# Herong1212/ORB_SLAM3_comments_ghr

Measured on AMD Instinct MI355X. Metric: Mmatches/s (256-bit Hamming), higher is better.
Workload: dtype fp4(e2m1)->f32; 1 GPU; C2: brute-force 256-bit Hamming top-2, 2000 x 2000 descriptors per frame, 1024 independent frames per launch per GPU (headline; the one-frame launch is `sing...; nq=2000, nt=2000, global_batch=1024, parallelism=replicas x1 (independent frames per GPU, no data-path collective)

## Files before the change

### orb_slam3_comments_ghr_amd/csrc/hamming_mfma.hip

```cpp
#include <algorithm>
#include <cstdlib>

#include "osg_internal.h"
#include "top2_key.h"
#include "top2_ring.h"

namespace {

typedef int i32x4 __attribute__((ext_vector_type(4)));
typedef int i32x16 __attribute__((ext_vector_type(16)));

constexpr int MF_PAD = 1 << 30;
constexpr int MF_RS = 272;

__device__ __forceinline__ int med3_i32(int a, int b, int c)
{
    return max(min(a, b), min(max(a, b), c));
}

__device__ __forceinline__ uint32_t spread_query(uint32_t nib)
{
    const uint32_t s = __umul24(nib, 0x204081u) & 0x01010101u;
    return ((0x80808080u - s) & 0x80808080u) | 0x40404040u;
}

__device__ __forceinline__ void key_push(int &k1, int &k2, int key)
{
    k2 = med3_i32(k1, key, k2);
    k1 = min(k1, key);
}

__device__ __forceinline__ void key_push2(int &k1, int &k2, int x, int y)
{
    const int m = med3_i32(k1, x, y);
    k1 = min(min(k1, x), y);
    k2 = min(m, k2);
}

__device__ __forceinline__ void key_push2f(int &k1, int &k2, int x, int y)
{
    const int m = __float_as_int(__builtin_amdgcn_fmed3f(__int_as_float(k1), __int_as_float(x), __int_as_float(y)));
    k1 = min(min(x, y), k1);
    k2 = min(m, k2);
}

__device__ __forceinline__ void key_merge(int &k1, int &k2, int a1, int a2)
{
    const int hi = max(k1, a1);
    k1 = min(k1, a1);
    k2 = min(min(k2, a2), hi);
}

template <int NW, int QT, int CR, int PIPE>
__global__ __launch_bounds__(NW * 64) void k_top2_mfma(const uint32_t *__restrict__ query, int nq,
                                                        const uint32_t *__restrict__ train, int nt,
                                                        int nqb, int32_t *__restrict__ out)
{
    constexpr int NT = NW * 64;
    constexpr int BPT = CR * 32 / NT;
    constexpr int WPT = BPT / 4;
    constexpr int TPR = 32 / BPT;
    constexpr int NTILE = CR / 32;
    static_assert(CR * 32 % NT == 0 && BPT % 4 == 0 && TPR >= 1, "chunk / workgroup shape");
    __shared__ __attribute__((aligned(16))) unsigned char s_buf[2 * CR * MF_RS];
    __shared__ uint2 s_lut[256];

    const int t = threadIdx.x, lane = t & 63;
    const int w = __builtin_amdgcn_readfirstlane(t >> 6);
    const int G = gridDim.x, L = blockIdx.x;
    const int logical = (G % 8 == 0) ? (L % 8) * (G / 8) + L / 8 : L;
    const int b = logical / nqb, qb = logical % nqb;
    const uint32_t *qf = query + (size_t)b * nq * 8;
    const uint32_t *tf = train + (size_t)b * nt * 8;
    int32_t *of = out + (size_t)b * nq * 3;

    for (int e = t; e < 256; e += NT) {
        uint32_t lo = 0, hi = 0;
#pragma unroll
        for (int y = 0; y < 4; y++) {
            lo |= ((e >> y) & 1u) << (8 * y + 7);
            hi |= ((e >> (y + 4)) & 1u) << (8 * y + 7);
        }
        s_lut[e] = make_uint2(lo, hi);
    }

    const int r = lane & 31, h = lane >> 5;
    const int qw0 = qb * (NW * QT * 32) + w * (QT * 32);
    const bool active = qw0 < nq;

    i32x4 bq[QT][8];
    int ka1[QT], ka2[QT], kb1[QT], kb2[QT], pq[QT];
#pragma unroll
    for (int j = 0; j < QT; j++) {
        const int q = min(qw0 + 32 * j + r, nq - 1);
        const uint4 lo = *(const uint4 *)(qf + (size_t)q * 8), hi = *(const uint4 *)(qf + (size_t)q * 8 + 4);
        const uint32_t wd[8] = {lo.x, lo.y, lo.z, lo.w, hi.x, hi.y, hi.z, hi.w};
        int pc = 0;
#pragma unroll
        for (int s = 0; s < 8; s++) {
            pc += __popc(wd[s]);
            const uint32_t hw = h ? (wd[s] >> 16) : (wd[s] & 0xFFFFu);
#pragma unroll
            for (int d = 0; d < 4; d++) bq[j][s][d] = (int)spread_query((hw >> (4 * d)) & 0xFu);
        }
        pq[j] = pc;
        ka1[j] = ka2[j] = kb1[j] = kb2[j] = (256 - pc) << MF_SHIFT;
    }
    i32x16 crow;
#pragma unroll
    for (int i = 0; i < 16; i++) crow[i] = (i & 3) + 8 * (i >> 2) + 4 * h;
    const int lbase = r * MF_RS + h * 16;

    const int erow = t / TPR, epart = t % TPR;
    auto load_chunk = [&](int c0, uint32_t (&pw)[WPT]) {
        const int row = c0 + erow;
        if (row < nt) {
            const uint32_t *src = tf + (size_t)row * 8 + epart * WPT;
#pragma unroll
            for (int i = 0; i < WPT; i += 2) {
                const uint2 v = *(const uint2 *)(src + i);
                pw[i] = v.x;
                pw[i + 1] = v.y;
            }
        } else {
#pragma unroll
            for (int i = 0; i < WPT; i++) pw[i] = 0u;
        }
    };
    auto store_chunk = [&](int buf, const uint32_t (&pw)[WPT]) {
        unsigned char *dst = s_buf + ((size_t)buf * CR + erow) * MF_RS;
#pragma unroll
        for (int i = 0; i < WPT; i++) {
#pragma unroll
            for (int hh = 0; hh < 2; hh++) {
                const int g = 2 * (epart * WPT + i) + hh;
                const uint2 v0 = s_lut[(pw[i] >> (16 * hh)) & 0xFFu];
                const uint2 v1 = s_lut[(pw[i] >> (16 * hh + 8)) & 0xFFu];
                *(i32x4 *)(dst + 16 * g) = i32x4{(int)v0.x, (int)v0.y, (int)v1.x, (int)v1.y};
            }
        }
    };

    auto frag = [&](const unsigned char *tb, int s) -> i32x4 { return *(const i32x4 *)(tb + lbase + 32 * s); };
    auto mfma = [&](const i32x4 &a, const i32x4 &bb, const i32x16 &c) {
        return __builtin_amdgcn_mfma_i32_32x32x32_i8(a, bb, c, 0, 0, 0);
    };
    auto epi = [&](const i32x16 (&acc)[QT]) {
#pragma unroll
        for (int j = 0; j < QT; j++) {
#pragma unroll
            for (int i = 0; i < 8; i += 2) {
                key_push2(ka1[j], ka2[j], acc[j][i], acc[j][i + 1]);
                key_push2(kb1[j], kb2[j], acc[j][i + 8], acc[j][i + 9]);
            }
            ka1[j] -= 32;
            ka2[j] -= 32;
            kb1[j] -= 32;
            kb2[j] -= 32;
        }
    };
    auto tile = [&](const unsigned char *tb, const i32x16 &cin) {
        i32x4 a[8];
#pragma unroll
        for (int s = 0; s < 8; s++) a[s] = frag(tb, s);
        i32x16 acc[QT];
#pragma unroll
        for (int j = 0; j < QT; j++) acc[j] = mfma(a[0], bq[j][0], cin);
#pragma unroll
        for (int s = 1; s < 8; s++)
#pragma unroll
            for (int j = 0; j < QT; j++) acc[j] = mfma(a[s], bq[j][s], acc[j]);
        epi(acc);
    };

    const int nch = (nt + CR - 1) / CR;
    {
        uint32_t pw[WPT];
        load_chunk(0, pw);
        __syncthreads();
        store_chunk(0, pw);
    }
    __syncthreads();
    for (int c = 0; c < nch; c++) {
        const int c0 = c * CR;
        uint32_t pw[WPT];
        const bool more = c + 1 < nch;
        if (more) load_chunk(c0 + CR, pw);
        if (active) {
            const unsigned char *sb = s_buf + (size_t)(c & 1) * CR * MF_RS;
            const int nfull = min(NTILE, (nt - c0) / 32);
            if (PIPE && nfull == NTILE) {
                i32x4 a[8];
                i32x16 accp[QT], acc[QT];
#pragma unroll
                for (int s = 0; s < 8; s++) a[s] = frag(sb, s);
#pragma unroll
                for (int s = 0; s < 8; s++) {
#pragma unroll
                    for (int j = 0; j < QT; j++) accp[j] = mfma(a[s], bq[j][s], s ? accp[j] : crow);
                    a[s] = frag(sb + 32 * MF_RS, s);
                    __builtin_amdgcn_sched_barrier(0);
                }
#pragma unroll
                for (int tt = 1; tt < NTILE; tt++) {
#pragma unroll
                    for (int s = 0; s < 8; s++) {
#pragma unroll
                        for (int j = 0; j < QT; j++) acc[j] = mfma(a[s], bq[j][s], s ? acc[j] : crow);
                        if (tt + 1 < NTILE) a[s] = frag(sb + (tt + 1) * 32 * MF_RS, s);
#pragma unroll
                        for (int j = 0; j < QT; j++) {
                            if (s & 1)
                                key_push2(kb1[j], kb2[j], accp[j][8 + (s & 6)], accp[j][9 + (s & 6)]);
                            else
                                key_push2(ka1[j], ka2[j], accp[j][s & 6], accp[j][1 + (s & 6)]);
                            if (s == 7) {
                                ka1[j] -= 32;
                                ka2[j] -= 32;
                                kb1[j] -= 32;
                                kb2[j] -= 32;
                            }
                        }
                        __builtin_amdgcn_sched_barrier(0);
                    }
#pragma unroll
                    for (int j = 0; j < QT; j++) accp[j] = acc[j];
                }
                epi(accp);
            } else {
#pragma unroll
                for (int tt = 0; tt < NTILE; tt++) {
                    if (tt >= nfull) break;
                    tile(sb + tt * 32 * MF_RS, crow);
                }
            }
            const int lim = nt - (c0 + nfull * 32);
            if (nfull < NTILE && lim > 0) {
                i32x16 cin;
#pragma unroll
                for (int i = 0; i < 16; i++) cin[i] = crow[i] + (crow[i] >= lim ? MF_PAD : 0);
                tile(sb + nfull * 32 * MF_RS, cin);
            }
        }
        if (more) store_chunk((c + 1) & 1, pw);
        __syncthreads();
    }
    if (!active) return;
    const int base = 32 * ((nt + 31) / 32);
#pragma unroll
    for (int j = 0; j < QT; j++) {
        int k1 = ka1[j], k2 = ka2[j];
        key_merge(k1, k2, kb1[j], kb2[j]);
        const int a1 = __shfl_xor(k1, 32), a2 = __shfl_xor(k2, 32);
        key_merge(k1, k2, a1, a2);
        const int q = qw0 + 32 * j + r;
        if (h == 0 && q < nq) {
            const int t1 = k1 + base, t2 = k2 + base;
            const int d1 = (t1 >> MF_SHIFT) + pq[j], d2 = (t2 >> MF_SHIFT) + pq[j];
            of[3 * q + 0] = d1 < 256 ? (t1 & (MF_MAX_ROWS - 1)) : -1;
            of[3 * q + 1] = min(d1, 256);
            of[3 * q + 2] = min(d2, 256);
        }
    }
}

constexpr int MX_RS = 144;
constexpr int MX_SCALE_TRAIN = 127 + 12;
constexpr int MX_SCALE_ONE = 127;
constexpr float MX_BIAS = 10485760.0f;
constexpr float MX_PAD = 1073741824.0f;

typedef int i32x8 __attribute__((ext_vector_type(8)));
typedef float f32x16 __attribute__((ext_vector_type(16)));

__device__ __forceinline__ uint32_t spread_nib(uint32_t x)
{
    x &= 0xFFu;
    x = (x | (x << 12)) & 0x000F000Fu;
    x = (x | (x << 6)) & 0x03030303u;
    return (x | (x << 3)) & 0x11111111u;
}

__device__ __forceinline__ uint32_t spread_nib9(uint32_t x)
{
    uint32_t lo3 = x * 0x40201u;
    asm("" : "+v"(lo3));
    return (lo3 | (x << 27)) & 0x88888888u;
}

template <int NW, int QT, int CR, int PIPE>
__global__ __launch_bounds__(NW * 64) void k_top2_fp4(const uint32_t *__restrict__ query, int nq,
                                                       const uint32_t *__restrict__ train, int nt,
                                                       int nqb, int32_t *__restrict__ out)
{
    constexpr int NT = NW * 64;
    constexpr int BPT = CR * 32 / NT;
    constexpr int WPT = BPT / 4;
    constexpr int TPR = 32 / BPT;
    constexpr int NTILE = CR / 32;
    static_assert(CR * 32 % NT == 0 && BPT % 4 == 0 && TPR >= 1, "chunk / workgroup shape");
    __shared__ __attribute__((aligned(16))) unsigned char s_buf[2 * CR * MX_RS];
    __shared__ uint32_t s_lut[256];

    const int t = threadIdx.x, lane = t & 63;
    const int w = __builtin_amdgcn_readfirstlane(t >> 6);
    const int G = gridDim.x, L = blockIdx.x;
    const int logical = (G % 8 == 0) ? (L % 8) * (G / 8) + L / 8 : L;
    const int b = logical / nqb, qb = logical % nqb;
    const uint32_t *qf = query + (size_t)b * nq * 8;
    const uint32_t *tf = train + (size_t)b * nt * 8;
    int32_t *of = out + (size_t)b * nq * 3;

    for (int e = t; e < 256; e += NT) s_lut[e] = spread_nib((uint32_t)e) * 0xCu;

    const int r = lane & 31, h = lane >> 5;
    const int qw0 = qb * (NW * QT * 32) + w * (QT * 32);
    const bool active = qw0 < nq;

    i32x8 bq[QT][4];
    int ka1[QT], ka2[QT], kb1[QT], kb2[QT];
    constexpr bool ONE = PIPE == 3 || PIPE == 4 || PIPE == 5;
    constexpr bool PART = PIPE == 5;
    int(&kc1)[QT] = ONE ? ka1 : kb1;
    int(&kc2)[QT] = ONE ? ka2 : kb2;
    int pq[QT];
#pragma unroll
    for (int j = 0; j < QT; j++) {
        const int q = min(qw0 + 32 * j + r, nq - 1);
        const uint4 lo = *(const uint4 *)(qf + (size_t)q * 8), hi = *(const uint4 *)(qf + (size_t)q * 8 + 4);
        const uint32_t wd[8] = {lo.x, lo.y, lo.z, lo.w, hi.x, hi.y, hi.z, hi.w};
        int pc = 0;
#pragma unroll
        for (int k = 0; k < 8; k++) pc += __popc(wd[k]);
#pragma unroll
        for (int s = 0; s < 4; s++) {
            const uint32_t word = wd[2 * s + h];
#pragma unroll
            for (int d = 0; d < 4; d++)
                bq[j][s][d] = (int)(0x22222222u | ((~spread_nib(word >> (8 * d)) & 0x11111111u) << 3));
#pragma unroll
            for (int d = 4; d < 8; d++) bq[j][s][d] = 0;
        }
        pq[j] = pc;
        ka1[j] = ka2[j] = kb1[j] = kb2[j] = ((256 - pc) << MF_SHIFT) + MX_KEY0;
    }
    f32x16 crow;
#pragma unroll
    for (int i = 0; i < 16; i++) crow[i] = MX_BIAS + (float)((i & 3) + 8 * (i >> 2) + 4 * h);
    const int lbase = r * MX_RS + h * 16;

    const int erow = t / TPR, epart = t % TPR;
    auto load_chunk = [&](int c0, uint32_t (&pw)[WPT]) {
        const int row = c0 + erow;
        if (row < nt) {
            const uint32_t *src = tf + (size_t)row * 8 + epart * WPT;
#pragma unroll
            for (int i = 0; i < WPT; i += 2) {
                const uint2 v = *(const uint2 *)(src + i);
                pw[i] = v.x;
                pw[i + 1] = v.y;
            }
        } else {
#pragma unroll
            for (int i = 0; i < WPT; i++) pw[i] = 0u;
        }
    };
    auto store_chunk = [&](int buf, const uint32_t (&pw)[WPT]) {
        unsigned char *dst = s_buf + ((size_t)buf * CR + erow) * MX_RS;
#pragma unroll
        for (int i = 0; i < WPT; i++) {
            const uint32_t x = pw[i];
            *(i32x4 *)(dst + 16 * (epart * WPT + i)) =
                i32x4{(int)s_lut[x & 0xFFu], (int)s_lut[(x >> 8) & 0xFFu], (int)s_lut[(x >> 16) & 0xFFu],
                      (int)s_lut[x >> 24]};
        }
    };

    auto frag = [&](const unsigned char *tb, int s) -> i32x8 {
        const i32x4 v = *(const i32x4 *)(tb + lbase + 32 * s);
        return i32x8{v[0], v[1], v[2], v[3], 0, 0, 0, 0};
    };
    auto mfma = [&](const i32x8 &a, const i32x8 &bb, const f32x16 &c) {
        return __builtin_amdgcn_mfma_scale_f32_32x32x64_f8f6f4(a, bb, c, 4, 4, 0, MX_SCALE_TRAIN, 0, MX_SCALE_ONE);
    };
    auto epi = [&](const f32x16 (&acc)[QT]) {
#pragma unroll
        for (int j = 0; j < QT; j++) {
#pragma unroll
            for (int i = 0; i < 8; i += 2) {
                key_push2f(ka1[j], ka2[j], __float_as_int(acc[j][i]), __float_as_int(acc[j][i + 1]));
                key_push2f(kc1[j], kc2[j], __float_as_int(acc[j][i + 8]), __float_as_int(acc[j][i + 9]));
            }
            ka1[j] -= 32;
            ka2[j] -= 32;
            if (!ONE) {
                kb1[j] -= 32;
                kb2[j] -= 32;
            }
        }
    };
    auto tile = [&](const unsigned char *tb, const f32x16 &cin) {
        i32x8 a[4];
#pragma unroll
        for (int s = 0; s < 4; s++) a[s] = frag(tb, s);
        f32x16 acc[QT];
#pragma unroll
        for (int j = 0; j < QT; j++) acc[j] = mfma(a[0], bq[j][0], cin);
#pragma unroll
        for (int s = 1; s < 4; s++)
#pragma unroll
            for (int j = 0; j < QT; j++) acc[j] = mfma(a[s], bq[j][s], acc[j]);
        epi(acc);
    };

    const int nch = (nt + CR - 1) / CR;
    {
        uint32_t pw[WPT];
        load_chunk(0, pw);
        __syncthreads();
        store_chunk(0, pw);
    }
    __syncthreads();
    for (int c = 0; c < nch; c++) {
        const int c0 = c * CR;
        uint32_t pw[WPT];
        const bool more = c + 1 < nch;
        if (more) load_chunk(c0 + CR, pw);
        if (active) {
            const unsigned char *sb = s_buf + (size_t)(c & 1) * CR * MX_RS;
            const int nfull = min(NTILE, (nt - c0) / 32);
            if (PIPE && (nfull == NTILE || (PART && nfull >= 1))) {
                i32x8 a[4];
                f32x16 accp[QT], acc[QT];
#pragma unroll
                for (int s = 0; s < 4; s++) a[s] = frag(sb, s);
#pragma unroll
                for (int s = 0; s < 4; s++) {
#pragma unroll
                    for (int j = 0; j < QT; j++) accp[j] = mfma(a[s], bq[j][s], s ? accp[j] : crow);
                    a[s] = frag(sb + 32 * MX_RS, s);
                    __builtin_amdgcn_sched_barrier(0);
                }
#pragma unroll
                for (int tt = 1; tt < NTILE; tt++) {
                    if (PART && tt >= nfull) break;
#pragma unroll
                    for (int s = 0; s < 4; s++) {
#pragma unroll
                        for (int j = 0; j < QT; j++) acc[j] = mfma(a[s], bq[j][s], s ? acc[j] : crow);
                        if (tt + 1 < NTILE) a[s] = frag(sb + (tt + 1) * 32 * MX_RS, s);
                        if (PIPE == 4) {
                            if (s == 1) {
                                bool need = false;
#pragma unroll
                                for (int j = 0; j < QT; j++) {
                                    int m = __float_as_int(accp[j][0]);
#pragma unroll
                                    for (int e = 1; e < 16; e += 2)
                                        m = min(min(m, __float_as_int(accp[j][e])),
                                                __float_as_int(accp[j][e + 1 < 16 ? e + 1 : e]));
                                    need |= m < ka2[j];
                                }
                                if (__builtin_amdgcn_ballot_w64(need) != 0) {
#pragma unroll
                                    for (int j = 0; j < QT; j++)
#pragma unroll
                                        for (int e = 0; e < 16; e += 2)
                                            key_push2f(ka1[j], ka2[j], __float_as_int(accp[j][e]),
                                                      __float_as_int(accp[j][e + 1]));
                                }
#pragma unroll
                                for (int j = 0; j < QT; j++) {
                                    ka1[j] -= 32;
                                    ka2[j] -= 32;
                                }
                            }
                            __builtin_amdgcn_sched_barrier(0);
                            continue;
                        }
#pragma unroll
                        for (int j = 0; j < QT; j++) {
                            if (PIPE == 2) {
#pragma unroll
                                for (int p = 0; p < 8; p++) {
                                    if (p / 3 + 1 != s) continue;
                                    const int e = (p & 3) * 2 + (p >> 2) * 8;
                                    if (p < 4) key_push2f(ka1[j], ka2[j], __float_as_int(accp[j][e]), __float_as_int(accp[j][e + 1]));
                                    else key_push2f(kb1[j], kb2[j], __float_as_int(accp[j][e]), __float_as_int(accp[j][e + 1]));
                                }
                            } else {
                                key_push2f(ka1[j], ka2[j], __float_as_int(accp[j][2 * s]),
                                          __float_as_int(accp[j][2 * s + 1]));
                                key_push2f(kc1[j], kc2[j], __float_as_int(accp[j][8 + 2 * s]),
                                          __float_as_int(accp[j][9 + 2 * s]));
                            }
                            if (s == 3) {
                                ka1[j] -= 32;
                                ka2[j] -= 32;
                                if (!ONE) {
                                    kb1[j] -= 32;
                                    kb2[j] -= 32;
                                }
                            }
                        }
                        __builtin_amdgcn_sched_barrier(0);
                    }
#pragma unroll
                    for (int j = 0; j < QT; j++) accp[j] = acc[j];
                }
                epi(accp);
            } else {
#pragma unroll
                for (int tt = 0; tt < NTILE; tt++) {
                    if (tt >= nfull) break;
                    tile(sb + tt * 32 * MX_RS, crow);
                }
            }
            const int lim = nt - (c0 + nfull * 32);
            if (nfull < NTILE && lim > 0) {
                f32x16 cin;
#pragma unroll
                for (int i = 0; i < 16; i++)
                    cin[i] = crow[i] + ((i & 3) + 8 * (i >> 2) + 4 * h >= lim ? MX_PAD : 0.f);
                tile(sb + nfull * 32 * MX_RS, cin);
            }
        }
        if (more) store_chunk((c + 1) & 1, pw);
        __syncthreads();
    }
    if (!active) return;
    const int base = 32 * ((nt + 31) / 32);
#pragma unroll
    for (int j = 0; j < QT; j++) {
        int k1 = ka1[j], k2 = ka2[j];
        if (!ONE) key_merge(k1, k2, kb1[j], kb2[j]);
        const int a1 = __shfl_xor(k1, 32), a2 = __shfl_xor(k2, 32);
        key_merge(k1, k2, a1, a2);
        const int q = qw0 + 32 * j + r;
        if (h == 0 && q < nq) {
            const int t1 = k1 - MX_KEY0 + base, t2 = k2 - MX_KEY0 + base;
            const int d1 = (t1 >> MF_SHIFT) + pq[j], d2 = (t2 >> MF_SHIFT) + pq[j];
            of[3 * q + 0] = d1 < 256 ? (t1 & (MF_MAX_ROWS - 1)) : -1;
            of[3 * q + 1] = min(d1, 256);
            of[3 * q + 2] = min(d2, 256);
        }
    }
}

template <int NW, int QT, int CR>
__global__ __launch_bounds__(NW * 64) void k_top2_fp4p(const uint32_t *__restrict__ query, int nq,
                                                        const uint32_t *__restrict__ train, int nt,
                                                        int nqb, int n_items, int32_t *__restrict__ out)
{
    constexpr int NT = NW * 64;
    constexpr int BPT = CR * 32 / NT;
    constexpr int WPT = BPT / 4;
    constexpr int TPR = 32 / BPT;
    constexpr int NTILE = CR / 32;
    static_assert(CR * 32 % NT == 0 && BPT % 4 == 0 && TPR >= 1, "chunk / workgroup shape");
    __shared__ __attribute__((aligned(16))) unsigned char s_buf[2 * CR * MX_RS];
    __shared__ uint32_t s_lut[256];

    const int t = threadIdx.x, lane = t & 63;
    const int w = __builtin_amdgcn_readfirstlane(t >> 6);
    const int G = gridDim.x;
    auto logical_of = [&](int item) { return (n_items % 8 == 0) ? (item % 8) * (n_items / 8) + item / 8 : item; };
    int item = blockIdx.x;
    if (item >= n_items) return;
    for (int e = t; e < 256; e += NT) s_lut[e] = spread_nib((uint32_t)e) * 0xCu;
    const int r = lane & 31, h = lane >> 5;
    const int lbase = r * MX_RS + h * 16;
    const int erow = t / TPR, epart = t % TPR;
    auto load_chunk = [&](const uint32_t *tfp, int c0, uint32_t (&pw)[WPT]) {
        const int row = c0 + erow;
        if (row < nt) {
            const uint32_t *src = tfp + (size_t)row * 8 + epart * WPT;
#pragma unroll
            for (int i = 0; i < WPT; i += 2) {
                const uint2 v = *(const uint2 *)(src + i);
                pw[i] = v.x;
                pw[i + 1] = v.y;
            }
        } else {
#pragma unroll
            for (int i = 0; i < WPT; i++) pw[i] = 0u;
        }
    };
    auto store_chunk = [&](int buf, const uint32_t (&pw)[WPT]) {
        unsigned char *dst = s_buf + ((size_t)buf * CR + erow) * MX_RS;
#pragma unroll
        for (int i = 0; i < WPT; i++) {
            const uint32_t x = pw[i];
            *(i32x4 *)(dst + 16 * (epart * WPT + i)) =
                i32x4{(int)s_lut[x & 0xFFu], (int)s_lut[(x >> 8) & 0xFFu], (int)s_lut[(x >> 16) & 0xFFu],
                      (int)s_lut[x >> 24]};
        }
    };
    auto frag = [&](const unsigned char *tb, int s) -> i32x8 {
        const i32x4 v = *(const i32x4 *)(tb + lbase + 32 * s);
        return i32x8{v[0], v[1], v[2], v[3], 0, 0, 0, 0};
    };
    auto mfma = [&](const i32x8 &a, const i32x8 &bb, const f32x16 &c) {
        return __builtin_amdgcn_mfma_scale_f32_32x32x64_f8f6f4(a, bb, c, 4, 4, 0, MX_SCALE_TRAIN, 0, MX_SCALE_ONE);
    };
    const int nch = (nt + CR - 1) / CR;
    {
        uint32_t pw[WPT];
        load_chunk(train + (size_t)(logical_of(item) / nqb) * nt * 8, 0, pw);
        __syncthreads();
        store_chunk(0, pw);
    }
    __syncthreads();
    int bufbase = 0;
    for (; item < n_items; item += G) {
        const int logical = logical_of(item);
        const int b = logical / nqb, qb = logical % nqb;
        const uint32_t *qf = query + (size_t)b * nq * 8;
        const uint32_t *tf = train + (size_t)b * nt * 8;
        int32_t *of = out + (size_t)b * nq * 3;
        const int next = item + G;
        const uint32_t *tfn = next < n_items ? train + (size_t)(logical_of(next) / nqb) * nt * 8 : nullptr;
        const int qw0 = qb * (NW * QT * 32) + w * (QT * 32);
        const bool active = qw0 < nq;
        i32x8 bq[QT][4];
        int ka1[QT], ka2[QT], pq[QT];
#pragma unroll
        for (int j = 0; j < QT; j++) {
            const int q = min(qw0 + 32 * j + r, nq - 1);
            const uint4 lo = *(const uint4 *)(qf + (size_t)q * 8), hi = *(const uint4 *)(qf + (size_t)q * 8 + 4);
            const uint32_t wd[8] = {lo.x, lo.y, lo.z, lo.w, hi.x, hi.y, hi.z, hi.w};
            int pc = 0;
#pragma unroll
            for (int k = 0; k < 8; k++) pc += __popc(wd[k]);
#pragma unroll
            for (int s = 0; s < 4; s++) {
                const uint32_t word = wd[2 * s + h];
#pragma unroll
                for (int d = 0; d < 4; d++)
                    bq[j][s][d] = (int)(0x22222222u | ((~spread_nib(word >> (8 * d)) & 0x11111111u) << 3));
#pragma unroll
                for (int d = 4; d < 8; d++) bq[j][s][d] = 0;
            }
            pq[j] = pc;
            ka1[j] = ka2[j] = ((256 - pc) << MF_SHIFT) + MX_KEY0;
        }
        f32x16 crow;
#pragma unroll
        for (int i = 0; i < 16; i++) crow[i] = MX_BIAS + (float)((i & 3) + 8 * (i >> 2) + 4 * h);
        auto epi = [&](const f32x16 (&acc)[QT]) {
#pragma unroll
            for (int j = 0; j < QT; j++) {
#pragma unroll
                for (int i = 0; i < 8; i += 2) {
                    key_push2f(ka1[j], ka2[j], __float_as_int(acc[j][i]), __float_as_int(acc[j][i + 1]));
                    key_push2f(ka1[j], ka2[j], __float_as_int(acc[j][i + 8]), __float_as_int(acc[j][i + 9]));
                }
                ka1[j] -= 32;
                ka2[j] -= 32;
            }
        };
        auto tile = [&](const unsigned char *tb, const f32x16 &cin) {
            i32x8 a[4];
#pragma unroll
            for (int s = 0; s < 4; s++) a[s] = frag(tb, s);
            f32x16 acc[QT];
#pragma unroll
            for (int j = 0; j < QT; j++) acc[j] = mfma(a[0], bq[j][0], cin);
#pragma unroll
            for (int s = 1; s < 4; s++)
#pragma unroll
                for (int j = 0; j < QT; j++) acc[j] = mfma(a[s], bq[j][s], acc[j]);
            epi(acc);
        };
        for (int c = 0; c < nch; c++) {
            const int c0 = c * CR;
            uint32_t pw[WPT];
            const bool more_in = c + 1 < nch, more = more_in || tfn != nullptr;
            if (more_in) load_chunk(tf, c0 + CR, pw);
            else if (tfn) load_chunk(tfn, 0, pw);
            if (active) {
                const unsigned char *sb = s_buf + (size_t)((c + bufbase) & 1) * CR * MX_RS;
                const int nfull = min(NTILE, (nt - c0) / 32);
                if (nfull == NTILE) {
                    i32x8 a[4];
                    f32x16 accp[QT], acc[QT];
#pragma unroll
                    for (int s = 0; s < 4; s++) a[s] = frag(sb, s);
#pragma unroll
                    for (int s = 0; s < 4; s++) {
#pragma unroll
                        for (int j = 0; j < QT; j++) accp[j] = mfma(a[s], bq[j][s], s ? accp[j] : crow);
                        a[s] = frag(sb + 32 * MX_RS, s);
                        __builtin_amdgcn_sched_barrier(0);
                    }
#pragma unroll
                    for (int tt = 1; tt < NTILE; tt++) {
#pragma unroll
                        for (int s = 0; s < 4; s++) {
#pragma unroll
                            for (int j = 0; j < QT; j++) acc[j] = mfma(a[s], bq[j][s], s ? acc[j] : crow);
                            if (tt + 1 < NTILE) a[s] = frag(sb + (tt + 1) * 32 * MX_RS, s);
#pragma unroll
                            for (int j = 0; j < QT; j++) {
                                key_push2f(ka1[j], ka2[j], __float_as_int(accp[j][2 * s]),
                                           __float_as_int(accp[j][2 * s + 1]));
                                key_push2f(ka1[j], ka2[j], __float_as_int(accp[j][8 + 2 * s]),
                                           __float_as_int(accp[j][9 + 2 * s]));
                                if (s == 3) {
                                    ka1[j] -= 32;
                                    ka2[j] -= 32;
                                }
                            }
                            __builtin_amdgcn_sched_barrier(0);
                        }
#pragma unroll
                        for (int j = 0; j < QT; j++) accp[j] = acc[j];
                    }
                    epi(accp);
                } else {
#pragma unroll
                    for (int tt = 0; tt < NTILE; tt++) {
                        if (tt >= nfull) break;
                        tile(sb + tt * 32 * MX_RS, crow);
                    }
                }
                const int lim = nt - (c0 + nfull * 32);
                if (nfull < NTILE && lim > 0) {
                    f32x16 cin;
#pragma unroll
                    for (int i = 0; i < 16; i++)
                        cin[i] = crow[i] + ((i & 3) + 8 * (i >> 2) + 4 * h >= lim ? MX_PAD : 0.f);
                    tile(sb + nfull * 32 * MX_RS, cin);
                }
            }
            if (more) store_chunk((c + 1 + bufbase) & 1, pw);
            __syncthreads();
        }
        bufbase = (bufbase + nch) & 1;
        if (active) {
            const int base = 32 * ((nt + 31) / 32);
#pragma unroll
            for (int j = 0; j < QT; j++) {
                int k1 = ka1[j], k2 = ka2[j];
                const int a1 = __shfl_xor(k1, 32), a2 = __shfl_xor(k2, 32);
                key_merge(k1, k2, a1, a2);
                const int q = qw0 + 32 * j + r;
                if (h == 0 && q < nq) {
                    const int t1 = k1 - MX_KEY0 + base, t2 = k2 - MX_KEY0 + base;
                    const int d1 = (t1 >> MF_SHIFT) + pq[j], d2 = (t2 >> MF_SHIFT) + pq[j];
                    of[3 * q + 0] = d1 < 256 ? (t1 & (MF_MAX_ROWS - 1)) : -1;
                    of[3 * q + 1] = min(d1, 256);
                    of[3 * q + 2] = min(d2, 256);
                }
            }
        }
    }
}

template <int NW, int CR>
__global__ __launch_bounds__(NW * 64) void k_top2_fp4q2(const uint32_t *__restrict__ query, int nq,
                                                         const uint32_t *__restrict__ train, int nt,
                                                         int nqb, int32_t *__restrict__ out)
{
    constexpr int NT = NW * 64;
    constexpr int BPT = CR * 32 / NT;
    constexpr int WPT = BPT / 4;
    constexpr int TPR = 32 / BPT;
    constexpr int NTILE = CR / 32;
    static_assert(CR * 32 % NT == 0 && BPT % 8 == 0 && TPR >= 1, "chunk / workgroup shape");
    constexpr int SLOTB = CR * MX_RS;
    __shared__ __attribute__((aligned(16))) unsigned char s_mem[1024 + TOP2_RING_SLOTS * SLOTB];
    uint32_t *const s_lut = (uint32_t *)s_mem;
    unsigned char *const s_buf = s_mem + 1024;

    const int t = threadIdx.x, lane = t & 63;
    const int w = __builtin_amdgcn_readfirstlane(t >> 6);
    const int G = gridDim.x, L = blockIdx.x;
    const int logical = (G % 8 == 0) ? (L % 8) * (G / 8) + L / 8 : L;
    const int b = logical / nqb, qb = logical % nqb;
    const uint32_t *qf = query + (size_t)b * nq * 8;
    const uint32_t *tf = train + (size_t)b * nt * 8;
    int32_t *of = out + (size_t)b * nq * 3;

    for (int e = t; e < 256; e += NT) {
        const uint32_t x = spread_nib9((uint32_t)e);
        s_lut[e] = x | (x >> 1);
    }

    const int r = lane & 31, h = lane >> 5;
    const int qw0 = qb * (NW * 64) + w * 64;
    const bool act0 = qw0 < nq, act1 = qw0 + 32 < nq;

    auto load_chunk = [&](int t, int c0, uint32_t (&pw)[WPT]) {
        const char *src = (const char *)tf + (c0 + t / TPR < nt ? (unsigned)((c0 * 8 + t * WPT) * 4) : 0u);
#pragma unroll
        for (int i = 0; i < WPT; i += 2) {
            const uint2 v = *(const uint2 *)(src + 4 * i);
            pw[i] = v.x;
            pw[i + 1] = v.y;
        }
    };
    uint32_t pw[WPT], p1[WPT];
    load_chunk(t, 0, pw);
    load_chunk(t, CR, p1);

    i32x8 bq[2][4];
    int k1[2], k2[2];
#pragma unroll
    for (int j = 0; j < 2; j++) {
        const int q = min(qw0 + 32 * j + r, nq - 1);
        const uint4 lo = *(const uint4 *)(qf + (size_t)q * 8), hi = *(const uint4 *)(qf + (size_t)q * 8 + 4);
        const int pc = __popc(lo.x) + __popc(lo.y) + __popc(lo.z) + __popc(lo.w) + __popc(hi.x) + __popc(hi.y) +
                       __popc(hi.z) + __popc(hi.w);
        const uint32_t wsel[4] = {h ? lo.y : lo.x, h ? lo.w : lo.z, h ? hi.y : hi.x, h ? hi.w : hi.z};
#pragma unroll
        for (int s = 0; s < 4; s++) {
            const uint32_t word = wsel[s];
#pragma unroll
            for (int d = 0; d < 4; d++)
                bq[j][s][d] = (int)(spread_nib9((word >> (8 * d)) & 0xFFu) ^ 0xAAAAAAAAu);
#pragma unroll
            for (int d = 4; d < 8; d++) bq[j][s][d] = 0;
        }
        k1[j] = k2[j] = ((256 - pc) << MF_SHIFT) + MX_KEY0;
    }
    f32x16 crow;
#pragma unroll
    for (int i = 0; i < 16; i++) crow[i] = MX_BIAS + (float)((i & 3) + 8 * (i >> 2) + 4 * h);
    int lbase = r * MX_RS + h * 16;

    auto store_chunk = [&](int t, int buf, int c0, const uint32_t (&pw)[WPT]) {
        const bool in = c0 + t / TPR < nt;
        unsigned char *dst = s_buf + buf * SLOTB + ((t & (NT - 1)) / TPR) * MX_RS + (t % TPR) * (16 * WPT);
#pragma unroll
        for (int i = 0; i < WPT; i++) {
            const uint32_t x = in ? pw[i] : 0u;
            *(i32x4 *)(dst + 16 * i) =
                i32x4{(int)s_lut[x & 0xFFu], (int)s_lut[(x >> 8) & 0xFFu], (int)s_lut[(x >> 16) & 0xFFu],
                      (int)s_lut[x >> 24]};
        }
    };
    auto frag = [&](const unsigned char *tb, int s) -> i32x8 {
        const i32x4 v = *(const i32x4 *)(tb + lbase + 32 * s);
        return i32x8{v[0], v[1], v[2], v[3], 0, 0, 0, 0};
    };
    auto mfma = [&](const i32x8 &a, const i32x8 &bb, const f32x16 &c) {
        return __builtin_amdgcn_mfma_scale_f32_32x32x64_f8f6f4(a, bb, c, 4, 4, 0, MX_SCALE_TRAIN, 0, MX_SCALE_ONE);
    };
    auto push = [&](int j, const f32x16 &acc, int s) {
        key_push2f(k1[j], k2[j], __float_as_int(acc[2 * s]), __float_as_int(acc[2 * s + 1]));
        key_push2f(k1[j], k2[j], __float_as_int(acc[8 + 2 * s]), __float_as_int(acc[9 + 2 * s]));
        if (s == 3) k1[j] -= TOP2_TILE_ROWS;
    };
    auto pushk = [&](int j, const f32x16 &acc, int s) {
        const int lo = s == 0 ? 0 : 3 * (s - 1), hi = s == 0 ? 0 : (s == 3 ? 8 : 3 * s);
#pragma unroll
        for (int p = lo; p < hi; p++) {
            const int e = (p & 1) * 8 + 2 * (p >> 1);
            key_push2f(k1[j], k2[j], __float_as_int(acc[e]), __float_as_int(acc[e + 1]));
        }
        if (s == 3) k1[j] -= TOP2_TILE_ROWS;
    };
    auto tile = [&](const unsigned char *tb, const f32x16 &cin) {
        i32x8 a[4];
#pragma unroll
        for (int s = 0; s < 4; s++) a[s] = frag(tb, s);
        f32x16 acc0 = mfma(a[0], bq[0][0], cin);
#pragma unroll
        for (int s = 1; s < 4; s++) acc0 = mfma(a[s], bq[0][s], acc0);
        if (act1) {
            f32x16 acc1 = mfma(a[0], bq[1][0], cin);
#pragma unroll
            for (int s = 1; s < 4; s++) acc1 = mfma(a[s], bq[1][s], acc1);
#pragma unroll
            for (int s = 0; s < 4; s++) push(0, acc0, s);
#pragma unroll
            for (int s = 0; s < 4; s++) push(1, acc1, s);
        } else {
#pragma unroll
            for (int s = 0; s < 4; s++) push(0, acc0, s);
        }
    };

    const int nch = top2_ring_chunks(nt, CR), nfc = top2_ring_full_chunks(nt, CR);
    __syncthreads();
    store_chunk(t, top2_ring_slot(0), 0, pw);
    store_chunk(t, top2_ring_slot(1), CR, p1);
    load_chunk(t, TOP2_RING_AHEAD * CR, pw);
    __syncthreads();
    auto lane_again = [&]() {
        int ln;
        asm volatile("v_mbcnt_lo_u32_b32 %0, -1, 0\n\tv_mbcnt_hi_u32_b32 %0, -1, %0" : "=v"(ln));
        return ln & 63;
    };
    auto seam = [&](int c, int freed) {
        __syncthreads();
        const int ln = lane_again(), tv = w * 64 + ln;
        store_chunk(tv, freed, (c + TOP2_RING_AHEAD) * CR, pw);
        load_chunk(tv, (c + TOP2_RING_AHEAD + 1) * CR, pw);
        return ln;
    };
    int slot = top2_ring_slot(0), freed = top2_ring_slot(TOP2_RING_SLOTS - 1);
    if (act1) {
        if (nfc > 0) {
            i32x8 a[4];
            f32x16 acc0, acc1;
#pragma unroll
            for (int s = 0; s < 4; s++) a[s] = frag(s_buf + slot * SLOTB, s);
#pragma unroll
            for (int i = 0; i < 16; i++) acc1[i] = MX_PAD;
            k1[1] += TOP2_TILE_ROWS;
            for (int c = 0; c < nfc; c++) {
#pragma unroll
                for (int s = 0; s < 4; s++) {
                    acc0 = mfma(a[s], bq[0][s], s ? acc0 : crow);
                    __builtin_amdgcn_sched_barrier(0);
                    pushk(1, acc1, s);
                    __builtin_amdgcn_sched_barrier(0);
                }
                const int ln = seam(c, freed);
                const int next = top2_ring_next(slot);
                lbase = (ln & 31) * MX_RS + (ln >> 5) * 16;
                const unsigned char *sb = s_buf + slot * SLOTB, *sn = sb + (next - slot) * SLOTB;
#pragma unroll
                for (int tt = 0; tt < NTILE; tt++) {
                    const unsigned char *nb = tt + 1 < NTILE ? sb + (tt + 1) * 32 * MX_RS : sn;
#pragma unroll
                    for (int s = 0; s < 4; s++) {
                        acc1 = mfma(a[s], bq[1][s], s ? acc1 : crow);
                        a[s] = frag(nb, s);
                        __builtin_amdgcn_sched_barrier(0);
                        pushk(0, acc0, s);
                        __builtin_amdgcn_sched_barrier(0);
                    }
                    if (tt + 1 == NTILE) break;
#pragma unroll
                    for (int s = 0; s < 4; s++) {
                        acc0 = mfma(a[s], bq[0][s], s ? acc0 : crow);
                        __builtin_amdgcn_sched_barrier(0);
                        pushk(1, acc1, s);
                        __builtin_amdgcn_sched_barrier(0);
                    }
                }
                freed = slot;
                slot = next;
            }
#pragma unroll
            for (int s = 0; s < 4; s++) push(1, acc1, s);
        }
    } else {
        for (int c = 0; c < nfc; c++) {
            seam(c, freed);
            if (act0) {
                const int nfull = min(NTILE, (nt - c * CR) / 32);
#pragma unroll 1
                for (int tt = 0; tt < nfull; tt++) tile(s_buf + slot * SLOTB + tt * 32 * MX_RS, crow);
            }
            freed = slot;
            slot = top2_ring_next(slot);
        }
    }
    if (nfc < nch) {
        seam(nfc, freed);
        if (act0) {
            const int ln = (int)__builtin_amdgcn_mbcnt_hi(~0u, __builtin_amdgcn_mbcnt_lo(~0u, 0u)), h = ln >> 5;
            lbase = (ln & 31) * MX_RS + h * 16;
            const unsigned char *sb = s_buf + slot * SLOTB;
            const int c0 = nfc * CR, nfull = (nt - c0) / 32;
#pragma unroll 1
            for (int tt = 0; tt < nfull; tt++) tile(sb + tt * 32 * MX_RS, crow);
            const int lim = nt - (c0 + nfull * 32);
            if (lim > 0) {
                f32x16 cin;
#pragma unroll
                for (int i = 0; i < 16; i++)
                    cin[i] = crow[i] + (4 * h >= lim - ((i & 3) + 8 * (i >> 2)) ? MX_PAD : 0.f);
                tile(sb + nfull * 32 * MX_RS, cin);
            }
        }
    }
    if (!act0) return;
    const int base = 32 * ((nt + 31) / 32);
    const int lane_end = (int)__builtin_amdgcn_mbcnt_hi(~0u, __builtin_amdgcn_mbcnt_lo(~0u, 0u));
#pragma unroll
    for (int j = 0; j < 2; j++) {
        int m1 = k1[j], m2 = k2[j];
        const int a1 = __shfl_xor(m1, 32), a2 = __shfl_xor(m2, 32);
        m2 = min(min(m2, a2), max(m1, a1) + TOP2_K2_LAST_REBASE);
        m1 = min(m1, a1);
        const int q = qw0 + 32 * j + lane_end;
        if (lane_end < 32 && q < nq) {
            const uint4 lo = *(const uint4 *)(qf + (size_t)q * 8), hi = *(const uint4 *)(qf + (size_t)q * 8 + 4);
            const int pc = __popc(lo.x) + __popc(lo.y) + __popc(lo.z) + __popc(lo.w) + __popc(hi.x) + __popc(hi.y) +
                           __popc(hi.z) + __popc(hi.w);
            const int d1 = top2_k1_dist(m1, base) + pc, d2 = top2_k2_dist(m2) + pc;
            of[3 * q + 0] = d1 < 256 ? top2_k1_row(m1, base) : -1;
            of[3 * q + 1] = min(d1, 256);
            of[3 * q + 2] = min(d2, 256);
        }
    }
}

template <int NW, int CR>
int launch_fp4q2(osg_ctx *ctx, const void *d_query, int nq, const void *d_train, int nt, int nb, void *d_out)
{
    const int nqb = (nq + NW * 64 - 1) / (NW * 64);
    const long long g = (long long)nqb * nb;
    OSG_REQUIRE(ctx, g <= 0x7FFFFFFF, "grid too large");
    hipLaunchKernelGGL((k_top2_fp4q2<NW, CR>), dim3((unsigned)g), dim3(NW * 64), 0, ctx->stream,
                       (const uint32_t *)d_query, nq, (const uint32_t *)d_train, nt, nqb, (int32_t *)d_out);
    OSG_HIP_CHECK(ctx, hipGetLastError());
    return OSG_OK;
}

template <int NW, int QT, int CR>
int launch_fp4p(osg_ctx *ctx, const void *d_query, int nq, const void *d_train, int nt, int nb, void *d_out)
{
    const int nqb = (nq + NW * QT * 32 - 1) / (NW * QT * 32);
    const long long items = (long long)nqb * nb;
    OSG_REQUIRE(ctx, items <= 0x7FFFFFFF, "grid too large");
    static int ncu = 0;
    if (ncu == 0) {
        int dev = 0, n = 0;
        if (hipGetDevice(&dev) == hipSuccess && hipDeviceGetAttribute(&n, hipDeviceAttributeMultiprocessorCount, dev) == hipSuccess && n > 0)
            ncu = n;
        else
            ncu = 256;
    }
    const int g = (int)std::min<long long>(items, ncu);
    hipLaunchKernelGGL((k_top2_fp4p<NW, QT, CR>), dim3((unsigned)std::max(g, 1)), dim3(NW * 64), 0, ctx->stream,
                       (const uint32_t *)d_query, nq, (const uint32_t *)d_train, nt, nqb, (int)items, (int32_t *)d_out);
    OSG_HIP_CHECK(ctx, hipGetLastError());
    return OSG_OK;
}

template <int NW, int QT, int CR, int PIPE>
int launch_fp4(osg_ctx *ctx, const void *d_query, int nq, const void *d_train, int nt, int nb, void *d_out)
{
    const int nqb = (nq + NW * QT * 32 - 1) / (NW * QT * 32);
    const long long g = (long long)nqb * nb;
    OSG_REQUIRE(ctx, g <= 0x7FFFFFFF, "grid too large");
    hipLaunchKernelGGL((k_top2_fp4<NW, QT, CR, PIPE>), dim3((unsigned)g), dim3(NW * 64), 0, ctx->stream,
                       (const uint32_t *)d_query, nq, (const uint32_t *)d_train, nt, nqb, (int32_t *)d_out);
    OSG_HIP_CHECK(ctx, hipGetLastError());
    return OSG_OK;
}

template <int NW, int QT, int CR, int PIPE>
int launch(osg_ctx *ctx, const void *d_query, int nq, const void *d_train, int nt, int nb, void *d_out)
{
    const int nqb = (nq + NW * QT * 32 - 1) / (NW * QT * 32);
    const long long g = (long long)nqb * nb;
    OSG_REQUIRE(ctx, g <= 0x7FFFFFFF, "grid too large");
    hipLaunchKernelGGL((k_top2_mfma<NW, QT, CR, PIPE>), dim3((unsigned)g), dim3(NW * 64), 0, ctx->stream,
                       (const uint32_t *)d_query, nq, (const uint32_t *)d_train, nt, nqb, (int32_t *)d_out);
    OSG_HIP_CHECK(ctx, hipGetLastError());
    return OSG_OK;
}

}

int osg_top2_mfma_max_rows() { return MF_MAX_ROWS; }

namespace {
int mfma_shape()
{
    static const int shape = getenv("OSG_TOP2_MFMA_SHAPE") ? atoi(getenv("OSG_TOP2_MFMA_SHAPE")) : 0;
    return shape;
}
bool mfma_fp4()
{
    static const bool fp4 = !(getenv("OSG_TOP2_FP4") && atoi(getenv("OSG_TOP2_FP4")) == 0);
    return fp4;
}
void mfma_shape_of(bool fp4, int shape, int *d)
{
    static const int i8[5][4] = {{16, 1, 256, 1}, {8, 2, 256, 1}, {16, 1, 256, 0}, {8, 2, 256, 0}, {8, 1, 256, 1}};
    static const int f4[14][4] = {{16, 1, 256, 3}, {8, 2, 256, 1}, {16, 1, 256, 0}, {16, 1, 256, 3}, {8, 1, 256, 1},
                                  {16, 2, 256, 1}, {16, 1, 256, 2}, {16, 1, 256, 1}, {16, 1, 256, 4}, {8, 1, 256, 3},
                                  {16, 1, 512, 3}, {16, 1, 256, 5}, {16, 1, 512, 5}, {16, 1, 256, 6}};
    const int *s = fp4 ? f4[(shape >= 1 && shape <= 13 && shape != 3) ? shape : 0]
                       : i8[(shape >= 1 && shape <= 4) ? shape : 0];
    for (int i = 0; i < 4; i++) d[i] = s[i];
}
bool mfma_q2(bool fp4, int shape) { return fp4 && !(shape >= 1 && shape <= 13); }
}

int osg_hamming_top2_batch_plan(osg_ctx *ctx, int32_t nq, int32_t nt, int32_t nb, char *name, int32_t len)
{
    if (!ctx || !name || len <= 0) return OSG_E_INVALID;
    const bool mf = getenv("OSG_TOP2_BATCH_MFMA") == nullptr || atoi(getenv("OSG_TOP2_BATCH_MFMA")) != 0;
    if (nq <= 0 || nb <= 0 || nt <= 0 || !mf || nt > MF_MAX_ROWS) {
        snprintf(name, (size_t)len, "%s", nq <= 0 || nb <= 0 ? "none" : "k_top2_batch");
        return OSG_OK;
    }
    if (mfma_q2(mfma_fp4(), mfma_shape())) {
        snprintf(name, (size_t)len, "k_top2_fp4q2<16,256> grid=%lld x %d", (long long)((nq + 1023) / 1024) * nb, 1024);
        return OSG_OK;
    }
    int d[4];
    mfma_shape_of(mfma_fp4(), mfma_shape(), d);
    const int per_wg = d[0] * d[1] * 32;
    snprintf(name, (size_t)len, "%s<%d,%d,%d,%d> grid=%lld x %d", mfma_fp4() ? "k_top2_fp4" : "k_top2_mfma", d[0], d[1],
             d[2], d[3], (long long)((nq + per_wg - 1) / per_wg) * nb, d[0] * 64);
    return OSG_OK;
}

int osg_launch_top2_batch_mfma(osg_ctx *ctx, const void *d_query, int32_t nq, const void *d_train, int32_t nt,
                               int32_t nb, void *d_out)
{
    OSG_REQUIRE(ctx, nt >= 1 && nt <= MF_MAX_ROWS, "nt=%d outside the MFMA path's 1..%d rows", nt, MF_MAX_ROWS);
    const int shape = mfma_shape();
    if (mfma_fp4()) {
        if (mfma_q2(true, shape)) return launch_fp4q2<16, 256>(ctx, d_query, nq, d_train, nt, nb, d_out);
        switch (shape) {
        case 1: return launch_fp4<8, 2, 256, 1>(ctx, d_query, nq, d_train, nt, nb, d_out);
        case 2: return launch_fp4<16, 1, 256, 0>(ctx, d_query, nq, d_train, nt, nb, d_out);
        case 4: return launch_fp4<8, 1, 256, 1>(ctx, d_query, nq, d_train, nt, nb, d_out);
        case 5: return launch_fp4<16, 2, 256, 1>(ctx, d_query, nq, d_train, nt, nb, d_out);
        case 6: return launch_fp4<16, 1, 256, 2>(ctx, d_query, nq, d_train, nt, nb, d_out);
        case 7: return launch_fp4<16, 1, 256, 1>(ctx, d_query, nq, d_train, nt, nb, d_out);
        case 8: return launch_fp4<16, 1, 256, 4>(ctx, d_query, nq, d_train, nt, nb, d_out);
        case 9: return launch_fp4<8, 1, 256, 3>(ctx, d_query, nq, d_train, nt, nb, d_out);
        case 10: return launch_fp4<16, 1, 512, 3>(ctx, d_query, nq, d_train, nt, nb, d_out);
        case 11: return launch_fp4<16, 1, 256, 5>(ctx, d_query, nq, d_train, nt, nb, d_out);
        case 12: return launch_fp4<16, 1, 512, 5>(ctx, d_query, nq, d_train, nt, nb, d_out);
        case 13: return launch_fp4p<16, 1, 256>(ctx, d_query, nq, d_train, nt, nb, d_out);
        default: return launch_fp4<16, 1, 256, 3>(ctx, d_query, nq, d_train, nt, nb, d_out);
        }
    }
    switch (shape) {
    case 1: return launch<8, 2, 256, 1>(ctx, d_query, nq, d_train, nt, nb, d_out);
    case 2: return launch<16, 1, 256, 0>(ctx, d_query, nq, d_train, nt, nb, d_out);
    case 3: return launch<8, 2, 256, 0>(ctx, d_query, nq, d_train, nt, nb, d_out);
    case 4: return launch<8, 1, 256, 1>(ctx, d_query, nq, d_train, nt, nb, d_out);
    default: return launch<16, 1, 256, 1>(ctx, d_query, nq, d_train, nt, nb, d_out);
    }
}
```

Before: 10.24 million Mmatches/s.

## Use buffer loads for train staging and peel non-prefetch tail chunks

Train-descriptor loads now go through AMD buffer resources whose size bound makes out-of-range reads return zero, so the per-thread bounds check and the zero-select in the store path go away. Staging offsets are precomputed once, the LDS lookup uses a scalar shift, and fragment addressing becomes an integer offset on a single running base instead of re-derived pointers and lane IDs. The main loop is specialised at compile time so the last chunks skip the useless store and prefetch. The MFMA scale operands are packed differently. This trims address and VALU work in the steady-state loop, but it relies on buffer out-of-bounds semantics and on the modified scale encoding staying equivalent.

```diff
diff --git a/orb_slam3_comments_ghr_amd/csrc/hamming_mfma.hip b/orb_slam3_comments_ghr_amd/csrc/hamming_mfma.hip
--- a/orb_slam3_comments_ghr_amd/csrc/hamming_mfma.hip
+++ b/orb_slam3_comments_ghr_amd/csrc/hamming_mfma.hip
@@ -1,5 +1,6 @@
 #include <algorithm>
 #include <cstdlib>
+#include <type_traits>
 
 #include "osg_internal.h"
 #include "top2_key.h"
@@ -791,18 +792,21 @@
     const int qw0 = qb * (NW * 64) + w * 64;
     const bool act0 = qw0 < nq, act1 = qw0 + 32 < nq;
 
-    auto load_chunk = [&](int t, int c0, uint32_t (&pw)[WPT]) {
-        const char *src = (const char *)tf + (c0 + t / TPR < nt ? (unsigned)((c0 * 8 + t * WPT) * 4) : 0u);
+    const unsigned src8 = (unsigned)t * (WPT * 4);
+    const int stg = (t / TPR) * MX_RS + (t % TPR) * (16 * WPT);
+    auto load_chunk = [&](unsigned src8, int c0, uint32_t (&pw)[WPT]) {
+        const __amdgpu_buffer_rsrc_t rs = __builtin_amdgcn_make_buffer_rsrc(
+            (void *)((const char *)tf + (size_t)c0 * 32), 0, max(nt - c0, 0) * 32, 0x00020000);
 #pragma unroll
         for (int i = 0; i < WPT; i += 2) {
-            const uint2 v = *(const uint2 *)(src + 4 * i);
+            const uint2 v = __builtin_bit_cast(uint2, __builtin_amdgcn_raw_buffer_load_b64(rs, (int)src8 + 4 * i, 0, 0));
             pw[i] = v.x;
             pw[i + 1] = v.y;
         }
     };
     uint32_t pw[WPT], p1[WPT];
-    load_chunk(t, 0, pw);
-    load_chunk(t, CR, p1);
+    load_chunk(src8, 0, pw);
+    load_chunk(src8, CR, p1);
 
     i32x8 bq[2][4];
     int k1[2], k2[2];
@@ -829,23 +833,24 @@
     for (int i = 0; i < 16; i++) crow[i] = MX_BIAS + (float)((i & 3) + 8 * (i >> 2) + 4 * h);
     int lbase = r * MX_RS + h * 16;
 
-    auto store_chunk = [&](int t, int buf, int c0, const uint32_t (&pw)[WPT]) {
-        const bool in = c0 + t / TPR < nt;
-        unsigned char *dst = s_buf + buf * SLOTB + ((t & (NT - 1)) / TPR) * MX_RS + (t % TPR) * (16 * WPT);
+    int two;
+    asm("s_mov_b32 %0, 2" : "=s"(two));
+    auto store_chunk = [&](int buf, const uint32_t (&pw)[WPT]) {
+        unsigned char *dst = s_buf + buf * SLOTB + stg;
 #pragma unroll
         for (int i = 0; i < WPT; i++) {
-            const uint32_t x = in ? pw[i] : 0u;
-            *(i32x4 *)(dst + 16 * i) =
-                i32x4{(int)s_lut[x & 0xFFu], (int)s_lut[(x >> 8) & 0xFFu], (int)s_lut[(x >> 16) & 0xFFu],
-                      (int)s_lut[x >> 24]};
-        }
-    };
-    auto frag = [&](const unsigned char *tb, int s) -> i32x8 {
-        const i32x4 v = *(const i32x4 *)(tb + lbase + 32 * s);
+            const uint32_t x = pw[i];
+            auto lut = [&](uint32_t byte) { return *(const int *)(s_mem + (byte << two)); };
+            *(i32x4 *)(dst + 16 * i) = i32x4{lut(x & 0xFFu), lut((x >> 8) & 0xFFu), lut((x >> 16) & 0xFFu), lut(x >> 24)};
+        }
+    };
+    auto frag = [&](int off, int s) -> i32x8 {
+        const i32x4 v = *(const i32x4 *)(s_buf + lbase + off + 32 * s);
         return i32x8{v[0], v[1], v[2], v[3], 0, 0, 0, 0};
     };
+    constexpr int MX_SCALES = MX_SCALE_TRAIN | (MX_SCALE_ONE << 8) | (MX_SCALE_ONE << 16);
     auto mfma = [&](const i32x8 &a, const i32x8 &bb, const f32x16 &c) {
-        return __builtin_amdgcn_mfma_scale_f32_32x32x64_f8f6f4(a, bb, c, 4, 4, 0, MX_SCALE_TRAIN, 0, MX_SCALE_ONE);
+        return __builtin_amdgcn_mfma_scale_f32_32x32x64_f8f6f4(a, bb, c, 4, 4, 0, MX_SCALES, 1, MX_SCALES);
     };
     auto push = [&](int j, const f32x16 &acc, int s) {
         key_push2f(k1[j], k2[j], __float_as_int(acc[2 * s]), __float_as_int(acc[2 * s + 1]));
@@ -861,7 +866,7 @@
         }
         if (s == 3) k1[j] -= TOP2_TILE_ROWS;
     };
-    auto tile = [&](const unsigned char *tb, const f32x16 &cin) {
+    auto tile = [&](int tb, const f32x16 &cin) {
         i32x8 a[4];
 #pragma unroll
         for (int s = 0; s < 4; s++) a[s] = frag(tb, s);
@@ -883,22 +888,18 @@
     };
 
     const int nch = top2_ring_chunks(nt, CR), nfc = top2_ring_full_chunks(nt, CR);
+    const int nex = min(nfc, max(nch - TOP2_RING_AHEAD, 0));
     __syncthreads();
-    store_chunk(t, top2_ring_slot(0), 0, pw);
-    store_chunk(t, top2_ring_slot(1), CR, p1);
-    load_chunk(t, TOP2_RING_AHEAD * CR, pw);
+    store_chunk(top2_ring_slot(0), pw);
+    store_chunk(top2_ring_slot(1), p1);
+    load_chunk(src8, TOP2_RING_AHEAD * CR, pw);
     __syncthreads();
-    auto lane_again = [&]() {
-        int ln;
-        asm volatile("v_mbcnt_lo_u32_b32 %0, -1, 0\n\tv_mbcnt_hi_u32_b32 %0, -1, %0" : "=v"(ln));
-        return ln & 63;
-    };
-    auto seam = [&](int c, int freed) {
+    auto seam = [&](int c, int freed, auto expand) {
         __syncthreads();
-        const int ln = lane_again(), tv = w * 64 + ln;
-        store_chunk(tv, freed, (c + TOP2_RING_AHEAD) * CR, pw);
-        load_chunk(tv, (c + TOP2_RING_AHEAD + 1) * CR, pw);
-        return ln;
+        if constexpr (decltype(expand)::value) {
+            store_chunk(freed, pw);
+            load_chunk(src8, (c + TOP2_RING_AHEAD + 1) * CR, pw);
+        }
     };
     int slot = top2_ring_slot(0), freed = top2_ring_slot(TOP2_RING_SLOTS - 1);
     if (act1) {
@@ -906,11 +907,11 @@
             i32x8 a[4];
             f32x16 acc0, acc1;
 #pragma unroll
-            for (int s = 0; s < 4; s++) a[s] = frag(s_buf + slot * SLOTB, s);
+            for (int s = 0; s < 4; s++) a[s] = frag(slot * SLOTB, s);
 #pragma unroll
             for (int i = 0; i < 16; i++) acc1[i] = MX_PAD;
             k1[1] += TOP2_TILE_ROWS;
-            for (int c = 0; c < nfc; c++) {
+            auto block = [&](int c, auto expand) {
 #pragma unroll
                 for (int s = 0; s < 4; s++) {
                     acc0 = mfma(a[s], bq[0][s], s ? acc0 : crow);
@@ -918,13 +919,12 @@
                     pushk(1, acc1, s);
                     __builtin_amdgcn_sched_barrier(0);
                 }
-                const int ln = seam(c, freed);
+                seam(c, freed, expand);
                 const int next = top2_ring_next(slot);
-                lbase = (ln & 31) * MX_RS + (ln >> 5) * 16;
-                const unsigned char *sb = s_buf + slot * SLOTB, *sn = sb + (next - slot) * SLOTB;
 #pragma unroll
                 for (int tt = 0; tt < NTILE; tt++) {
-                    const unsigned char *nb = tt + 1 < NTILE ? sb + (tt + 1) * 32 * MX_RS : sn;
+                    if (tt + 1 == NTILE) lbase += (next - slot) * SLOTB;
+                    const int nb = tt + 1 < NTILE ? (tt + 1) * 32 * MX_RS : 0;
 #pragma unroll
                     for (int s = 0; s < 4; s++) {
                         acc1 = mfma(a[s], bq[1][s], s ? acc1 : crow);
@@ -944,28 +944,33 @@
                 }
                 freed = slot;
                 slot = next;
-            }
+            };
+            int c = 0;
+            for (; c < nex; c++) block(c, std::true_type{});
+            if (c < nfc) block(c++, std::false_type{});
+            if (c < nfc) block(c++, std::false_type{});
 #pragma unroll
             for (int s = 0; s < 4; s++) push(1, acc1, s);
         }
     } else {
         for (int c = 0; c < nfc; c++) {
-            seam(c, freed);
+            if (c < nex) seam(c, freed, std::true_type{});
+            else seam(c, freed, std::false_type{});
             if (act0) {
                 const int nfull = min(NTILE, (nt - c * CR) / 32);
 #pragma unroll 1
-                for (int tt = 0; tt < nfull; tt++) tile(s_buf + slot * SLOTB + tt * 32 * MX_RS, crow);
+                for (int tt = 0; tt < nfull; tt++) tile(slot * SLOTB + tt * 32 * MX_RS, crow);
             }
             freed = slot;
             slot = top2_ring_next(slot);
         }
     }
     if (nfc < nch) {
-        seam(nfc, freed);
+        seam(nfc, freed, std::false_type{});
         if (act0) {
             const int ln = (int)__builtin_amdgcn_mbcnt_hi(~0u, __builtin_amdgcn_mbcnt_lo(~0u, 0u)), h = ln >> 5;
             lbase = (ln & 31) * MX_RS + h * 16;
-            const unsigned char *sb = s_buf + slot * SLOTB;
+            const int sb = slot * SLOTB;
             const int c0 = nfc * CR, nfull = (nt - c0) / 32;
 #pragma unroll 1
             for (int tt = 0; tt < nfull; tt++) tile(sb + tt * 32 * MX_RS, crow);
```

Result: faster. 10.42 million Mmatches/s (median of 6 runs) (+1.8%).
